# HKUST-Aerial-Robotics/VINS-Mono

Measured on AMD Instinct MI355X. Metric: sliding-window BA solves/sec (Estimator::optimization: 8-iteration dogleg solve + marginalization), higher is better.
Workload: dtype f64; 1 GPU; batch of 256 independent EuRoC-shape windows per step and GPU (K=11 frames, ~150 landmarks, 10 IMU factors, ~600 projection factors, 75-dim marginalization prior, max 8 iterations, MARGIN_OLD marginalization); windows resident in HBM; consecutive steps are issued to 16 HIP streams (independent batches in flight); windows_per_gpu=256, batches_in_flight=16, parallelism=independent batches x1 (no collectives)

## Files before the change

### vins-mono_amd/csrc/ba_host.hip

```cpp
#include "vg_range.h"
#include <hip/hip_runtime.h>
#include <algorithm>
#include <chrono>
#include <cmath>
#include <cstdio>
#include <cstdlib>
#include <cstring>
#include <string>
#include <thread>
#include <vector>
#include "ba_layout.h"
#include "vg_handle.h"
#include "../../include/vinsgpu.h"

struct BaFork { hipStream_t aux; hipEvent_t fork, join; };
extern "C" hipError_t ba_launch_solve(const BaLayout& L, const BaLayout* dL, const BaPtrs& P, int rounds, hipStream_t stream,
                                      hipEvent_t* ev, int* kinds, int* n_launches, const BaFork* fk);
typedef int (*BaAllReduce)(void* user, double* buf, size_t count, void* stream);
extern "C" hipError_t ba_launch_solve_big(const BaLayout& L, const BaLayout* dL, const BaPtrs& P, int rounds, int slack, hipStream_t stream,
                                          BaAllReduce allreduce, void* user, int* hook_rc, hipEvent_t* ev, int* kinds, int* n_launches);
extern "C" hipError_t ba_launch_eval_factors(const BaLayout& L, const BaLayout* dL, const BaPtrs& P, double* proj_r, double* proj_J,
                                            double* imu_r, double* imu_J, double* prior_r, hipStream_t stream);
extern "C" const char* ba_failed_launch();
extern "C" hipError_t ba_prepare_launch();
// ... 184 lines not shown
    }
    L.nbl = L.nbf + L.nig + L.nprw;
    {
        const int nb = L.Kp + L.e + L.t;
        L.ntask = nb * (nb + 1) / 2;
        const int per = BA_ACC_NT / 64;
        const int ng = L.e + L.t, nglob = ng * (ng + 1) / 2;
        L.nba = L.Kp + (ng ? 1 : 0) + (L.ntask - L.Kp - nglob + (L.Lcap + 63) / 64 + per - 1) / per;
    }
    int bigm_doubles = 0;
    {
        int ldc = L.RcPad;
        if ((2 * ldc) % 64 != 32) ldc += 16;
        L.ldc = ldc;
        int o = 0, ob = 0;
        int& oo = L.big ? ob : o;
        L.l_S = o; o += up((L.Rc + 1) * (L.Rc + 2) / 2, 2);
        L.l_XC = 0; L.l_ring = 0; L.l_pinv = 0;
        if (L.big) { L.l_XC = oo; oo += up(9 * L.K, 8) * ldc; }
        else {
            L.l_ring = o; o += 36 * ldc;
        }
        L.l_D = oo; oo += up(81 * L.K, 2);
        L.l_E = oo; oo += up(81 * L.K, 2);
        L.l_dinv = oo; oo += up(9 * L.K, 2);
        L.l_vec = oo; oo += 9 * L.Rpad;
        L.l_red = o; o += 32;
        if (L.big) { L.l_wd = oo; oo += up(std::max(9 * L.K, 162), 2); }
        else L.l_wd = L.l_ring;
        L.l_z = oo; oo += up(36 * L.K, 2);
        if (L.big) { L.l_pmap = oo; oo += up(L.Ncap, 4) / 2; }
        else { L.l_pmap = 0; L.l_pinv = o; o += up(L.R, 4) / 2; }
        if (L.big) { L.l_di = o; o += up(L.Rc + 1, 2); L.l_cz = o; o += 6 * 96; }
        L.l_Sg = 0;
        if (L.big) { L.l_Sg = oo; oo += up((L.Rc + 1) * (L.Rc + 2) / 2, 2); }
        L.lds_solve = o * 8;
        bigm_doubles = ob;
        if (!L.big && L.Rc + 10 - 64 > 32) { h->err = "solve kernel: more column tasks than three wavefronts"; return VG_ERR_UNSUPPORTED; }
        if (!L.big && 36 * ldc < std::max(std::max(L.RcPad * 33, 2 * SV_NT), std::max(9 * L.K, 162))) { h->err = "solve kernel: scratch does not fit the coupling-row ring"; return VG_ERR_UNSUPPORTED; }
        if (L.lds_solve > 160 * 1024) { h->err = "solve kernel LDS carve exceeds 160 KB"; return VG_ERR_UNSUPPORTED; }
        const int nib = std::min(std::min(L.K - 1, BA_IMU_BATCH), L.igs);
        L.lds_lin = 8 * std::max(up(nib * 225, 2) + nib * 480, 5 * L.Ncap);
        L.lds_pro = 8 * BA_NW * (L.imu_info ? 512 : 256);
        if (8 * L.Ncap * L.Ncap <= 128 * 1024) L.lds_pro = std::max(L.lds_pro, 8 * L.Ncap * L.Ncap);
        if (L.lds_lin > 128 * 1024) { h->err = "prior too large for the linearisation kernel"; return VG_ERR_UNSUPPORTED; }
        {
            static const bool env_off = getenv("VG_BA_FUSED") && !strcmp(getenv("VG_BA_FUSED"), "0");
            const bool off = env_off && !h->ba.no_env;
            static const int env_min = getenv("VG_BA_FUSED_MIN") ? atoi(getenv("VG_BA_FUSED_MIN")) : 32;
            const int la_min_windows = h->ba.fused_min >= 0 ? (h->ba.fused_min ? h->ba.fused_min : 1 << 30) : (env_min ? env_min : 1 << 30);
            const int npair = L.Kp * (L.Kp - 1) / 2;
            const int avail = (160 * 1024 - 8192 - 512) / 8;
            const int nstl = up(7 * L.Kp + 9 * L.K + 8, 2);
            int chf = (int)((avail - nstl - npair * 90 - 34 - (64 + 82 + 8 * 80) / 2) / 34.0);
            chf = std::min(chf & ~1, 512);
            L.la_on = (!off && L.nwin >= la_min_windows && !L.big && !L.e && !L.t && L.Kp <= 13 && chf >= 96 && (L.Fcap + chf - 17) / (chf - 16) <= 62) ? 1 : 0;
            L.la_chf = chf; L.la_chq = chf - 16;
            L.la_P = up(chf * 33, 2);
            L.la_key = L.la_P + up(npair * 90, 2);
            L.la_x = up(L.la_key + (2 * chf + 64 + 82 + 8 * 80 + 1) / 2 + 2, 2);
            L.lds_linacc = (L.la_x + nstl) * 8;
        }
        {
            static const int env_max = getenv("VG_BA_SOLVE_W8_BELOW") ? atoi(getenv("VG_BA_SOLVE_W8_BELOW")) : -1;
            const int below = (env_max >= 0 && !h->ba.no_env) ? env_max : 32;
            L.sv_w8 = (!L.big && L.nwin < below) ? 1 : 0;
            L.l_wd8 = L.lds_solve / 8;
            L.lds_solve_w8 = L.lds_solve + 8 * L.RcPad * 33;
            if (L.lds_solve_w8 > 160 * 1024) L.sv_w8 = 0;
        }
    }
    if (L.big) {
        const int nt = (L.Rc + 1 + 15) / 16;
        L.nts = nt * (nt + 1) / 2;
        const int ntri = L.Rc * (L.Rc + 1) / 2;
        L.rb1_T = up(ntri + L.Rc, 2);
        L.rb1_scal = L.rb1_T + up((L.Rc + 1) * (L.Rc + 2) / 2, 2);
        L.rb1_len = L.rb1_scal + RB1_NSCAL;
    }
    int o = 0;
    L.io_hdr = o; o += BA_HDR_INTS;
    L.io_lm_start = o; o += L.Lcap;
    L.io_lm_fbeg = o; o += L.Lcap + 8;
    L.io_fac_i = o; o += L.Fcap;
    L.io_fac_j = o; o += L.Fcap;
    L.io_fac_lm = o; o += L.Fcap;
    L.io_fac_oi = o; o += L.Fcap;
    L.io_fac_oj = o; o += L.Fcap;
    L.io_fac_slot = o; o += L.Fcap;
    L.io_pair_ptr = o; o += up(L.Kp * L.Kp + 1, 8);
    L.io_task_list = o; o += up(L.ntask, 8);
    L.io_imu_valid = o; o += up(L.K, 8);
    L.io_pb_kind = o; o += L.NBcap;
    L.io_pb_idx = o; o += L.NBcap;
    L.io_pb_col = o; o += L.NBcap;
    L.io_pb_off = o; o += L.NBcap;
    L.io_pb_x0off = o; o += L.NBcap;
    L.istride = up(o, 8);
    o = 0;
    L.do_pose = o; o += up(7 * L.Kp, 2);
    L.do_sb = o; o += up(9 * L.K, 2);
    L.do_ex = o; o += 8;
    L.do_td = o; o += 2;
    L.do_lam = o; o += L.Lcap;
    L.do_obs = o; o += L.Ocap * BA_OBS_STRIDE;
    L.do_imu = o; o += (L.K - 1) * BA_IMU_STRIDE;
    L.do_par = o; o += P_NPAR;
    L.dstride = up(o, 8);
    L.pld = std::max(up(6 * L.K + 9 * 2 + 6 + 1, 8), L.Ncap);
    L.po_x0 = 0;
    L.po_r0 = 9 * std::max(up(L.K + 4, 8), L.NBcap);
    L.po_J0 = L.po_r0 + L.pld;
    L.pstride = up(L.po_J0 + L.pld * L.pld, 8);
    o = 0;
    L.so_ctl = o; o += C_NCTL;
    L.so_part = o; o += up(L.nbl, 8);
    L.so_x = o; o += 2 * L.nst;
    L.so_lam = o; o += 2 * L.Lcap;
    L.so_imuU = o; o += up((L.K - 1) * 225, 2);
    L.so_Hp = o; o += L.Ncap * L.Ncap;
    L.so_J0t = o; o += L.Ncap * L.Ncap;
    L.so_rec = o; o += L.Fcap * L.REC;
    L.so_sc = o; o += L.Rpad;
    L.so_sl = o; o += L.Lcap;
    L.so_dg = o; o += L.Rpad + L.Lcap;
    L.so_gt = o; o += L.Rpad + L.Lcap;
    L.so_gn = o; o += L.Rpad + L.Lcap;
    L.so_yl = o; o += L.Lcap;
    L.so_lsc = o; o += L.Lcap;
    L.so_xp = 0;
    if (!L.big) { L.so_xp = o; o += up(9 * L.K, 4) * L.ldc; }
    if (L.big) {
        L.so_bigm = o; o += up(bigm_doubles, 8);
        L.so_dgl = o; o += 2 * L.Lcap;
        L.so_gtl = o; o += 2 * L.Lcap;
    }
    {
        int b = 0;
        L.bo_Sp = b; b += up(L.Rc * (L.Rc + 1) / 2, 2);
        L.bo_gp = b; b += L.RcPad;
        L.bo_h = b; b += L.Lcap;
        L.bo_b = b; b += L.Lcap;
        L.bo_Wt = b; b += L.RcPad * L.Lcap;
        L.bo_imuJ = b; b += (L.K - 1) * 512;
        L.bo_pr = b; b += L.Ncap;
        L.bo_gpr = b; b += L.Ncap;
        L.buf_stride = up(b, 8);
    }
    L.so_buf = o; o += 2 * L.buf_stride;
    L.sstride = up(o, 8);
    L.pl_off = (int)((sizeof(BaLayout) + 255) / 256 * 256);
    L.pl_n = L.big ? 0 : L.Rc * (L.Rc + 1) / 2 + L.Rpad + 2 * 81 * L.K;
    o = 0;
    L.oo_pose = o; o += up(7 * L.Kp, 2);
    L.oo_sb = o; o += up(9 * L.K, 2);
    L.oo_ex = o; o += 8;
    L.oo_td = o; o += 2;
    L.oo_lam = o; o += L.Lcap;
    L.oo_sum = o; o += BA_SUM_DOUBLES;
    L.oo_trace = o; o += 5 * VG_MAX_ITERS + 16;
    L.ostride = up(o, 8);
    L.oi_stride = up(4 + VG_MAX_ITERS, 8);
    L.mcap = up(6 * L.K + 9 * 2 + 6 + 1, 8);
    if (L.mcap > 256) { h->err = "kept dimension of the marginalization beyond the kernel's tables"; return VG_ERR_UNSUPPORTED; }
    const int mcap = L.mcap;
    L.mo_J0 = 0;
    L.mo_r0 = mcap * mcap;
    L.mo_x0 = L.mo_r0 + mcap;
    L.mo_stride = up(L.mo_x0 + (L.K + 4) * 9, 8);
    L.mi_stride = up(8 + 2 * (L.K + 4) + 16, 8);
    L.mg_posmax = up(mcap + 15 + L.Lcap, 2);
    {
        const int nstm = up(16 * L.K + 8 + 1, 2);
        L.mg_cs = up(std::max(std::max(2 * mcap, 3 * (L.mg_posmax / 2 + 2)), 2 * (3 * ((mcap + 2) / 2) + 2) + 2), 2);
        L.mg_cs = std::max(L.mg_cs, std::max(up(5 * mcap + 8, 2), up(L.Lcap + 512, 2)));
        const int fixed = 32 + nstm + BA_MARG_LDS_INTS / 2 + L.mg_cs;
        int ld = mcap + 1;
        while (2 * ld * ld + fixed > 160 * 1024 / 8) ld -= 2;
        L.mg_ld = ld;
        L.mg_lds_bytes = (2 * ld * ld + fixed) * 8;
        if (ld < 8) { h->err = "marginalization LDS carve failed"; return VG_ERR_UNSUPPORTED; }
        const long pm = L.mg_posmax;
        long sdoubles = pm * pm + pm + (long)L.Fcap * 42 + 2 * pm * (mcap + 1) + 2 * pm * pm + 2L * mcap * mcap + 2 * L.Ncap + 480 + L.Lcap + 64 + L.Lcap / 2 + 8;
        L.ms_stride = (int)up((int)sdoubles, 8);
    }
    return VG_OK;
}

struct FacTmp { int i, j, l, oi, oj; };

static int pack_window(vg_handle* h, const BaLayout& L, const vg_ba_problem* p, const PriorRef& pr, int margin, int* ia, double* di, double* hp) {
    const int K = L.K, Kp = L.Kp;
    int* hdr = ia + L.io_hdr;
    for (int o = 0; o < p->n_obs; ++o) {
        double* d = di + L.do_obs + (size_t)o * BA_OBS_STRIDE;
        for (int k = 0; k < 7; ++k) d[k] = p->obs[(size_t)o * 7 + k];
        d[7] = 0.0;
    }
    for (int k = 0; k < p->relo_n; ++k) {
        double* d = di + L.do_obs + (size_t)(p->n_obs + k) * BA_OBS_STRIDE;
        memset(d, 0, sizeof(double) * BA_OBS_STRIDE);
        d[0] = p->relo_xy[2 * k];
// ... 1385 lines not shown
```

### vins-mono_amd/csrc/ba_layout.h

```cpp
#pragma once

#ifndef BA_NT
#define BA_NT 512
#endif
#define BA_NW (BA_NT / 64)
#ifndef SV_NT
#define SV_NT 256
#endif
#define SV_NW (SV_NT / 64)
#define SV_WG_PER_CU (SV_NT <= 256 ? 2 : 1)
#define BA_LIN_NT 256
#define BA_ACC_NT 256
#define BA_MAX_K 13
#define BA_MAX_K_LARGE 40
#define BA_MARG_LDS_INTS 400
#ifndef BA_IMU_BATCH
#define BA_IMU_BATCH 16
#endif
#ifndef BA_IMU_GROUP
#define BA_IMU_GROUP 2
#endif
#define BA_IMU_STRIDE 472
#define BA_OBS_STRIDE 8
#define BA_SUM_DOUBLES 16
#define BA_HDR_INTS 16

enum { H_L = 0, H_F, H_NPRIOR, H_NBLK, H_MAXIT, H_NCHUNK, H_MARGIN, H_STATUS, H_MARGMODE };

enum {
    C_IT = 0, C_NACC, C_NINV, C_TERM, C_STATUS, C_RADIUS, C_MU, C_MUSOLVED, C_REUSE, C_COST, C_XNORM, C_ALPHA, C_GTN2,
    C_GNN2, C_GTGN, C_DNORM, C_MODEL, C_CUR, C_PENDING, C_DONE, C_STEPNORM, C_XNORMC, C_INITCOST, C_SCALED, C_QCAM,
    C_PHASE, C_GNN2C, C_GTGNC, C_STEP2C, C_XN2C,
    C_T0,
    C_TIMEDOUT,
    C_NCTL = 32
};

enum { RB1_COST = 0, RB1_GTL2, RB1_LAM2, RB1_STEP2, RB1_NBIG, RB1_NSCAL = 8 };
enum { RB2_GNN2 = 0, RB2_GTGN, RB2_QL, RB2_NONFIN };
#define BA_BIG_LM_BLOCKS 32
#define BA_BIG_ZERO_BLOCKS 8
#define RB2_LEN (4 * BA_BIG_LM_BLOCKS)

enum { V_G = 0, V_SC, V_DG, V_GT, V_GN, V_U, V_Y, V_T, V_DI, V_NVEC };
struct alignas(16) AsmPlanEntry { int dst, base, imu, cols; };

struct BaLayout {
    int nwin, K, Kp, e, t;
    int Rc, RcPad, R, Rpad;
    int Lcap, Fcap, Ocap, Ncap, NBcap;
    int REC;
    int nbf, nbl, nba, ntask;
    int nig, igs, nprw;
    int nst;
    int imu_info;
    int io_hdr, io_lm_start, io_lm_fbeg, io_fac_i, io_fac_j, io_fac_lm, io_fac_oi, io_fac_oj, io_fac_slot,
        io_pair_ptr, io_task_list, io_imu_valid, io_pb_kind, io_pb_idx, io_pb_col, io_pb_off, io_pb_x0off, istride;
    int do_pose, do_sb, do_ex, do_td, do_lam, do_obs, do_imu, do_par, dstride;
    int po_x0, po_r0, po_J0, pld, pstride;
    int so_ctl, so_part, so_x, so_lam;
    int so_imuU, so_Hp, so_rec;
    int so_J0t;
    int so_sc, so_sl, so_dg, so_gt, so_gn;
    int so_yl, so_lsc;
    int so_xp;
    int so_buf, buf_stride;
    int bo_Sp, bo_gp, bo_h, bo_b, bo_Wt, bo_imuJ, bo_pr, bo_gpr;
    int sstride;
    int oo_pose, oo_sb, oo_ex, oo_td, oo_lam, oo_sum, oo_trace, ostride;
    int oi_stride;
    int mo_J0, mo_r0, mo_x0, mo_stride;
    int mi_stride;
    int ms_stride;
    int mcap, mg_ld, mg_posmax, mg_cs, mg_lds_bytes;
    int l_S, l_XC, l_D, l_E, l_dinv, l_vec, l_red, l_wd, l_z, l_pmap, ldc, lds_solve;
    int l_ring, l_pinv;
    int pl_off, pl_n;
    int lds_lin, lds_pro;
    int la_on, la_chq, la_chf, la_P, la_key, la_x, lds_linacc;
    int sv_w8;
    int l_wd8, lds_solve_w8;
    int pro_split;
    int big;
    int so_bigm;
    int l_di, l_cz;
    int l_Sg;
    int so_dgl, so_gtl;
    int rb1_len, rb1_T, rb1_scal;
    int nts;
};

struct BaPtrs {
    int* iarr;
    double* din;
    double* scr;
    double* out;
    int* iout;
    double* mout;
    int* miout;
    double* mscr;
    double* rb1;
    double* rb2;
    double* pri;
};

enum { P_FOCAL = 0, P_TR, P_ROW, P_GNORM, P_MAXTIME, P_NPAR = 8 };
```

### vins-mono_amd/csrc/ba_pipeline.hip

```cpp
#include <hip/hip_runtime.h>
#include <vector>
#include <mutex>
#include <cstring>
#include <cstdlib>
#include "ba_layout.h"
#include "ba_factors.h"
#include "../../include/vinsgpu.h"

extern __shared__ __attribute__((aligned(16))) char bp_smem[];

#ifdef BA_SOLVE_W8_TU
#undef BA_PROFILE_DETAIL
#undef BA_DEBUG_DUMP
namespace vg_w8 {
#endif

#define NOINL __device__ __noinline__
#define AS_LDS(p) ((lds_d*)(p))
#define AS_LDS_C(p) ((const lds_d*)(p))
#define AS_GLB(p) ((glb_d*)(p))
#define AS_GLB_C(p) ((const glb_d*)(p))
#define AS_GLB_CI(p) ((const glb_i*)(p))
template <bool BIG> struct MovT { typedef lds_d D; typedef lds_i I; };
template <> struct MovT<true> { typedef glb_d D; typedef glb_i I; };
// ... 274 lines not shown
            for (int r = 0; r < 15; ++r) Uo[r * 15 + i] = (i >= r) ? A[i * 15 + r] : 0.0;
        __syncthreads();
    }
}

NOINL void imu_sqrt_info(const Ctx& c_in, int fbeg, int fend) {
    const Ctx c = c_in;
    const BaLayout L = *c.Lp;
    lds_d* A = AS_LDS(LDSB + c.wave * 256);
    const int nimu = fend < L.K - 1 ? fend : L.K - 1;
    const glb_i* valid = AS_GLB_CI(c.ia + L.io_imu_valid);
    const int li = c.lane < 15 ? c.lane : 14;
    for (int base = fbeg; base < nimu; base += BA_NW) {
        const int f = uni(base + c.wave);
        if (!(f < nimu && valid[f])) continue;
        const glb_d* cov = AS_GLB_C(c.di + L.do_imu + f * BA_IMU_STRIDE + IM_COV);
        double a[15];
#pragma unroll
        for (int k = 0; k < 15; ++k) a[k] = cov[li * 15 + k];
#pragma unroll
        for (int j = 14; j >= 0; --j) {
            const double d = sqrt(readlane_f64(a[j], j));
            a[j] = c.lane < j ? a[j] / d : (c.lane == j ? d : a[j]);
#pragma unroll
            for (int kk = 0; kk < j; ++kk) {
                const double ukj = readlane_f64(a[j], kk);
                a[kk] = (c.lane <= kk) ? a[kk] - a[j] * ukj : a[kk];
            }
        }
        if (c.lane < 15) {
#pragma unroll
            for (int k = 0; k < 15; ++k) A[c.lane * 15 + k] = a[k];
        }
        __builtin_amdgcn_wave_barrier();
        glb_d* Uo = AS_GLB(c.sc + L.so_imuU + f * 225);
        if (c.lane < 15) {
            const int j = c.lane;
            double x[15];
#pragma unroll
            for (int i = 14; i >= 0; --i) {
                double s = (i == j) ? 1.0 : 0.0;
#pragma unroll
                for (int k = 14; k > i; --k) s -= (k <= j) ? A[i * 15 + k] * x[k] : 0.0;
                x[i] = (i <= j) ? s / A[i * 15 + i] : 0.0;
            }
#pragma unroll
            for (int i = 0; i < 15; ++i) Uo[i * 15 + j] = x[i];
        }
        __builtin_amdgcn_wave_barrier();
    }
    __syncthreads();
}

#ifndef BA_SOLVE_W8_TU
extern "C" __global__ __launch_bounds__(BA_NT) void ba_prologue_kernel(const BaLayout* __restrict__ Lp, BaPtrs P) {
    const BaLayout& L = *Lp;
    Ctx c;
    ctx_init(c, Lp, P, blockIdx.x);
    double* x = c.sc + L.so_x;
    DP_DECL;
    const bool all = gridDim.y == 1;
    const int part = blockIdx.y, nI = (L.K - 1 + BA_NW - 1) / BA_NW;
    if (all || part == 0)
    {
        double* out = P.out + (size_t)blockIdx.x * L.ostride;
        int* iout = P.iout + (size_t)blockIdx.x * L.oi_stride;
        int* miout = P.miout + (size_t)blockIdx.x * L.mi_stride;
        for (int k = c.tid; k < L.ostride; k += BA_NT) out[k] = 0.0;
        for (int k = c.tid; k < L.oi_stride; k += BA_NT) iout[k] = 0;
        for (int k = c.tid; k < L.mi_stride; k += BA_NT) miout[k] = 0;
    }
    if (all || part == 0) {
        for (int k = c.tid; k < 7 * L.Kp; k += BA_NT) x[k] = c.di[L.do_pose + k];
        for (int k = c.tid; k < 9 * L.K; k += BA_NT) x[7 * L.Kp + k] = c.di[L.do_sb + k];
        if (c.tid < 7) x[7 * L.Kp + 9 * L.K + c.tid] = c.di[L.do_ex + c.tid];
        if (c.tid == 7) x[7 * L.Kp + 9 * L.K + 7] = c.di[L.do_td];
        for (int k = c.tid; k < c.nL; k += BA_NT) c.sc[L.so_lam + k] = c.di[L.do_lam + k];
        if (c.tid < C_NCTL) {
            double v = 0.0;
            if (c.tid == C_RADIUS) v = 1e4;
            if (c.tid == C_MU || c.tid == C_MUSOLVED) v = 1e-8;
            if (c.tid == C_T0) v = (double)wall_clock64();
            c.sc[L.so_ctl + c.tid] = v;
        }
    }
    DP_ADD(40);
    if (all || (part >= 1 && part <= nI)) {
        const int fbeg = all ? 0 : (part - 1) * BA_NW, fend = all ? L.K - 1 : part * BA_NW;
        if (L.imu_info) imu_sqrt_info_ref(c, fbeg, fend);
        else imu_sqrt_info(c, fbeg, fend);
    }
    DP_ADD(41);
    if (c.nprior && (all || part > nI)) {
        const bool do_copy = all || part == nI + 1, do_prod = all || part == nI + 2;
        const int n = c.nprior;
        const double* J0 = c.pri + L.po_J0;
        double* Hp = c.sc + L.so_Hp;
        if (do_copy) {
            double* J0t = c.sc + L.so_J0t;
            for (int wk = c.tid; wk < n * n; wk += BA_NT) { const int r = wk / n, cc = wk % n; J0t[cc * L.Ncap + r] = J0[r * L.pld + cc]; }
        }
        __syncthreads();
        DP_ADD(42);
        if (!do_prod) {
        } else if ((size_t)n * n * 8 <= (size_t)L.lds_pro) {
            double* J0s = LDSB;
            for (int wk = c.tid; wk < n * n; wk += BA_NT) J0s[wk] = J0[(wk / n) * L.pld + wk % n];
            __syncthreads();
            DP_ADD(43);
            const int T = (n + 15) >> 4, ntile = T * (T + 1) / 2, nks = (n + 3) >> 2;
            const int wave = c.tid >> 6, lane = c.tid & 63, li = lane & 15, lk = lane >> 4;
            for (int t = wave; t < ntile; t += BA_NT / 64) {
                int ta, tb;
                tri_decode(t, ta, tb);
                const int ca = 16 * ta + li, cb = 16 * tb + li;
                double4_t acc = (double4_t){0, 0, 0, 0};
                for (int ks = 0; ks < nks; ++ks) {
                    const int r = 4 * ks + lk;
                    const double av = (r < n && ca < n) ? J0s[r * n + ca] : 0.0;
                    const double bv = (r < n && cb < n) ? J0s[r * n + cb] : 0.0;
                    acc = __builtin_amdgcn_mfma_f64_16x16x4f64(av, bv, acc, 0, 0, 0);
                }
#pragma unroll
                for (int q = 0; q < 4; ++q) {
                    const int a = 16 * ta + lk + 4 * q, bb = 16 * tb + li;
                    if (a < n && bb <= a) {
                        Hp[a * L.Ncap + bb] = acc[q];
                    }
                }
            }
        } else {
            const int ld = L.pld;
            for (int wk = c.tid; wk < n * (n + 1) / 2; wk += BA_NT) {
                int a, bb;
                tri_decode(wk, a, bb);
                double s0 = 0.0, s1 = 0.0;
                int r = 0;
                for (; r + 1 < n; r += 2) { s0 += J0[r * ld + a] * J0[r * ld + bb]; s1 += J0[(r + 1) * ld + a] * J0[(r + 1) * ld + bb]; }
                if (r < n) s0 += J0[r * ld + a] * J0[r * ld + bb];
                Hp[a * L.Ncap + bb] = s0 + s1;
            }
        }
    }
    DP_ADD(44);
}
#endif

template <bool JAC>
NOINL double imu_pass(const Ctx& c_in, const double* x_, double* imuJ_, int fbeg, int fend) {
    const Ctx c = c_in;
    const BaLayout L = *c.Lp;
    const int nimu = fend;
    const glb_i* valid = AS_GLB_CI(c.ia + L.io_imu_valid);
    const glb_d* x = AS_GLB_C(x_);
    glb_d* imuJ = AS_GLB(imuJ_);
    const glb_d* gU = AS_GLB_C(c.sc + L.so_imuU);
    const int nb = fend - fbeg < BA_IMU_BATCH ? fend - fbeg : BA_IMU_BATCH;
    double* Us = LDSB;
    double* panels = Us + ((nb * 225 + 1) & ~1);
    double cost = 0.0;
    const int per = nb > BA_NW ? 2 : 1;
    const int half = c.lane >> 5, hl = c.lane & 31;
    for (int f0 = fbeg; f0 < nimu; f0 += nb) {
        const int nf = nimu - f0 < nb ? nimu - f0 : nb;
        for (int k0 = c.tid; k0 < nf * 225; k0 += 8 * BA_NT) {
            double uv[8];
#pragma unroll
            for (int u = 0; u < 8; ++u) { const int k = k0 + u * BA_NT; uv[u] = k < nf * 225 ? gU[f0 * 225 + k] : 0.0; }
#pragma unroll
            for (int u = 0; u < 8; ++u) { const int k = k0 + u * BA_NT; if (k < nf * 225) Us[k] = uv[u]; }
        }
        __syncthreads();
        const int fl = c.wave * per + half;
        const int f = f0 + fl;
        const bool act = fl < nf && half < per && valid[f];
        if (act) {
            const glb_d* pre = AS_GLB_C(c.di + L.do_imu + f * BA_IMU_STRIDE);
            double pi[7], si[9], pj[7], sj[9];
#pragma unroll
            for (int k = 0; k < 7; ++k) { pi[k] = x[7 * f + k]; pj[k] = x[7 * (f + 1) + k]; }
#pragma unroll
            for (int k = 0; k < 9; ++k) { si[k] = x[7 * L.Kp + 9 * f + k]; sj[k] = x[7 * L.Kp + 9 * (f + 1) + k]; }
            const double* U = Us + fl * 225;
            double* panel = panels + fl * 480;
            ImuCtx ic;
            imu_ctx<JAC>(pre, pi, si, pj, sj, c.gnorm, ic);
            double raw[15];
            if (JAC && hl < 30) imu_raw_col(ic, pre, hl, raw);
            else {
#pragma unroll
                for (int q = 0; q < 15; ++q) raw[q] = ic.r[q];
            }
            if (hl <= 30) {
#pragma unroll
                for (int r = 0; r < 15; ++r) {
                    double s = 0.0;
#pragma unroll
// ... 497 lines not shown
    buf[L.bo_b + l] = b;
    int row = 6 * L.Kp;
    if (L.e | L.t) {
        double wex[6] = {0, 0, 0, 0, 0, 0}, wtd = 0.0;
        const int otd = 28 + 12 * L.e;
        for (int f = fb; f < fe; ++f) {
            const double* rec = recs + (size_t)c.ia[L.io_fac_slot + f] * REC;
            const double l0 = rec[24], l1 = rec[25];
            if (L.e) {
#pragma unroll
                for (int k = 0; k < 6; ++k) wex[k] += rec[28 + 2 * k] * l0 + rec[28 + 2 * k + 1] * l1;
            }
            if (L.t) wtd += rec[otd] * l0 + rec[otd + 1] * l1;
        }
        if (L.e) {
#pragma unroll
            for (int k = 0; k < 6; ++k) Wt[(size_t)(col_ex(L) + k) * ldw] = anchor >= 0 ? wex[k] : 0.0;
            row += 6;
        }
        if (L.t) { Wt[(size_t)col_td(L) * ldw] = anchor >= 0 ? wtd : 0.0; row += 1; }
    }
    if (L.big) { Wt[row * ldw] = b; ++row; }
    for (; row < L.RcPad; ++row) Wt[row * ldw] = 0.0;
}

#ifndef BA_SOLVE_W8_TU
extern "C" __global__ __launch_bounds__(BA_ACC_NT) void ba_accumulate_kernel(const BaLayout* __restrict__ Lp, BaPtrs P) {
    const BaLayout& L = *Lp;
    const int bid = blockIdx.x;
    const int xcd = bid & 7, rest = bid >> 3;
    const int bx = rest % L.nba, w = (rest / L.nba) * 8 + xcd;
    if (w >= L.nwin) return;
    Ctx c;
    ctx_init(c, Lp, P, w);
    const double* ctl = c.sc + L.so_ctl;
    if (ctl[C_DONE] != 0.0) return;
    const int which = ((int)ctl[C_CUR]) ^ (ctl[C_PENDING] != 0.0 ? 1 : 0);
    double* buf = lin_buf(c, which);
    const double* recs = c.sc + L.so_rec;
    __shared__ double part[7 * 36 + 4];
    if (bx < L.Kp) { diag_pose_task(c, bx, recs, buf + L.bo_Sp, buf + L.bo_gp, part); return; }
    const int ng = L.e + L.t;
    if (ng && bx == L.Kp) { global_task(c, recs, buf + L.bo_Sp, buf + L.bo_gp, part); return; }
    const int g = (bx - L.Kp - (ng ? 1 : 0)) * (BA_ACC_NT / 64) + c.wave;
    const int nother = L.ntask - L.Kp - ng * (ng + 1) / 2;
    if (g < nother) owner_task(c, c.ia[L.io_task_list + g], c.lane, recs, buf + L.bo_Sp, buf + L.bo_gp);
    else {
        const int l = (g - nother) * 64 + c.lane;
        if (l < L.Lcap) landmark_task(c, l, recs, buf);
    }
}
#endif

#define LA_NT BA_NT
#define LA_RS 33
#define LA_NPW 6
#define LA_MAXP 13
#define LA_QCAP 80
static_assert(LA_QCAP <= 128, "the pair prefix of ba_linacc_proj_kernel takes two pairs per lane of one wavefront");
#define LA_PAIR 90
DEV int wave_scan_incl(int v) {
    v += __builtin_amdgcn_update_dpp(0, v, 0x111, 0xF, 0xF, true);
    v += __builtin_amdgcn_update_dpp(0, v, 0x112, 0xF, 0xF, true);
    v += __builtin_amdgcn_update_dpp(0, v, 0x114, 0xF, 0xF, true);
    v += __builtin_amdgcn_update_dpp(0, v, 0x118, 0xF, 0xF, true);
    const int r0 = __builtin_amdgcn_readlane(v, 15), r1 = __builtin_amdgcn_readlane(v, 31), r2 = __builtin_amdgcn_readlane(v, 47);
    const int row = (int)(threadIdx.x & 63) >> 4;
    return v + (row > 0 ? r0 : 0) + (row > 1 ? r1 : 0) + (row > 2 ? r2 : 0);
}
DEV int la_pair_q(int i, int j, int Kp) { const int d = j - i; return (d - 1) * Kp - (d - 1) * d / 2 + i; }
__device__ __forceinline__ void linacc_body(const BaLayout* __restrict__ Lp, const BaPtrs& P) {
    const BaLayout L = layout_load(Lp);
    Ctx c;
    ctx_init(c, Lp, P, blockIdx.x);
    const double* ctl = c.sc + L.so_ctl;
    if (ctl[C_DONE] != 0.0) return;
    const int which = uni(((int)ctl[C_CUR]) ^ (ctl[C_PENDING] != 0.0 ? 1 : 0));
    const double* x = c.sc + L.so_x + which * L.nst;
    const double* lam = c.sc + L.so_lam + which * L.Lcap;
    glb_d* buf = AS_GLB(lin_buf(c, which));
    const glb_i* ia = AS_GLB_CI(c.ia);
    lds_d* rec = AS_LDS(LDSB);
    lds_d* Pb = AS_LDS(LDSB + L.la_P);
    lds_i* key = (lds_i*)(LDSB + L.la_key);
    lds_i* lstart = key + L.la_chf;
    lds_i* posx = lstart + 64;
    lds_i* pstart = posx + L.la_chf;
    lds_i* wcnt = pstart + LA_QCAP + 2;
    __shared__ double red[2 * (LA_NT / 64)];
    const int Kp = L.Kp, npair = Kp * (Kp - 1) / 2, chq = L.la_chq;
    const int nL = c.nL;
    DP_DECL;
    {
        double share = 0.0;
        if (c.nprior > 0) {
            if (c.nprior * c.nprior <= 12 * LA_NT && 4 * L.Ncap <= 4 * LA_NT && (c.nprior * (c.nprior + 1) + 2 + 5 * L.Ncap) <= L.la_P)
                share = prior_staged(c, L, x, lin_buf(c, which) + L.bo_pr, lin_buf(c, which) + L.bo_gpr, LDSB);
            else
                share = prior_pass(c, x, lin_buf(c, which) + L.bo_pr, lin_buf(c, which) + L.bo_gpr, LDSB);
        }
        DP_ADD(23);
        share += imu_pass<true>(c, x, lin_buf(c, which) + L.bo_imuJ, 0, L.K - 1);
        const double tot_imu = block_sum(red, LA_NT / 64, c.lane, c.wave, share);
        for (int g = c.tid; g < L.nbl - L.nbf; g += LA_NT) c.sc[L.so_part + L.nbf + g] = g == 0 ? tot_imu : 0.0;
        __syncthreads();
        DP_ADD(22);
    }
    lds_d* xs = AS_LDS(LDSB + L.la_x);
    for (int k = c.tid; k < 7 * L.Kp + 9 * L.K + 8; k += LA_NT) xs[k] = AS_GLB_C(x)[k];
    const int nchunk = nL > 0 ? uni(ia[L.io_lm_fbeg + nL - 1] / chq + 1) : 0;
    for (int t = c.tid; t < nL; t += LA_NT) {
        const int cl = ia[L.io_lm_fbeg + t] / chq;
        if (t == 0 || ia[L.io_lm_fbeg + t - 1] / chq != cl) lstart[cl] = t;
    }
    if (c.tid == 0) lstart[nchunk] = nL;
    for (int e = c.tid; e < npair * LA_PAIR; e += LA_NT) Pb[e] = 0.0;
    const bool pair_wave = c.wave < LA_NPW;
    __syncthreads();
    DP_ADD(24);
    int pidx[4];
#pragma unroll
    for (int reg = 0; reg < 4; ++reg) {
        const int row = (c.lane >> 4) + 4 * reg, col = c.lane & 15;
        int idx = -1;
        if (row < 6) {
            if (col <= row) idx = row * (row + 1) / 2 + col;
            else if (col == 13) idx = 78 + row;
        } else if (row < 12) {
            if (col < 6) idx = 42 + (row - 6) * 6 + col;
            else if (col <= row && col < 12) idx = 21 + (row - 6) * (row - 5) / 2 + (col - 6);
            else if (col == 13) idx = 84 + (row - 6);
        }
        pidx[reg] = idx;
    }
    double cost = 0.0;
    for (int ch = 0; ch < nchunk; ++ch) {
        const int l0 = lstart[ch], l1 = lstart[ch + 1];
        const int f0 = ia[L.io_lm_fbeg + l0], f1 = ia[L.io_lm_fbeg + l1];
        const int nf = uni(f1 - f0);
        if (nf > L.la_chf) __builtin_trap();
        ProjIn pin;
        int q = -1, rank = 0;
        if (c.tid < nf) {
            proj_fetch_staged(c, f0 + c.tid, xs, lam, pin);
            q = la_pair_q(pin.i, pin.j, Kp);
        }
        for (int e = c.tid; e < (LA_NT / 64) * LA_QCAP; e += LA_NT) wcnt[e] = 0;
        __syncthreads();
        DP_ADD(45);
        {
            const unsigned long long act = __ballot(q >= 0);
            unsigned long long same = act;
#pragma unroll
            for (int b = 0; b < 7; ++b) {
                const bool bit = q >= 0 && ((q >> b) & 1);
                const unsigned long long mb = __ballot(bit);
                same &= bit ? mb : ~mb;
            }
            const unsigned long long lt = (1ull << c.lane) - 1ull;
            rank = __popcll(same & lt);
            if (q >= 0 && rank == 0) wcnt[c.wave * LA_QCAP + q] = __popcll(same);
        }
        __syncthreads();
        if (c.wave == 0) {
            int cw0[LA_NT / 64], cw1[LA_NT / 64];
            const int p0 = c.lane, p1 = c.lane + 64;
#pragma unroll
            for (int w = 0; w < LA_NT / 64; ++w) {
                cw0[w] = p0 < npair ? wcnt[w * LA_QCAP + p0] : 0;
                cw1[w] = p1 < npair ? wcnt[w * LA_QCAP + p1] : 0;
            }
            int t0 = 0, t1 = 0;
#pragma unroll
            for (int w = 0; w < LA_NT / 64; ++w) { const int a = cw0[w], b = cw1[w]; cw0[w] = t0; cw1[w] = t1; t0 += a; t1 += b; }
            const int i0 = wave_scan_incl(t0);
            const int tot0 = __builtin_amdgcn_readlane(i0, 63);
            const int i1 = wave_scan_incl(t1) + tot0;
            if (p0 < npair) {
                pstart[p0 + 1] = i0;
#pragma unroll
                for (int w = 0; w < LA_NT / 64; ++w) wcnt[w * LA_QCAP + p0] = i0 - t0 + cw0[w];
            }
            if (p1 < npair) {
                pstart[p1 + 1] = i1;
#pragma unroll
                for (int w = 0; w < LA_NT / 64; ++w) wcnt[w * LA_QCAP + p1] = i1 - t1 + cw1[w];
            }
            if (c.lane == 0) pstart[0] = 0;
        }
        __syncthreads();
        DP_ADD(46);
        if (c.tid < nf) {
            const int pos = wcnt[c.wave * LA_QCAP + q] + rank;
            double r[2], Ji[12], Jj[12], Jl[2];
            proj_eval<false, true, false>(pin.pi, pin.pj, pin.ex, pin.lam, pin.oi, pin.oj, 0.0, c.focal, c.tr, c.row, r, Ji, Jj, nullptr, Jl, nullptr);
            const double s = r[0] * r[0] + r[1] * r[1];
            const double sq = sqrt(1.0 / (1.0 + s));
            lds_d* qr = rec + pos * LA_RS;
#pragma unroll
            for (int k = 0; k < 6; ++k) {
                qr[k] = sq * Ji[k]; qr[16 + k] = sq * Ji[6 + k];
                qr[6 + k] = sq * Jj[k]; qr[22 + k] = sq * Jj[6 + k];
            }
            qr[12] = sq * Jl[0]; qr[28] = sq * Jl[1];
            qr[13] = sq * r[0]; qr[29] = sq * r[1];
            key[c.tid] = pin.i * 16 + pin.j;
            posx[c.tid] = pos;
            cost += log1p(s);
        }
        __syncthreads();
        DP_ADD(25);
        if (pair_wave) {
            double4_t acc[LA_MAXP];
#pragma unroll
            for (int k = 0; k < LA_MAXP; ++k) acc[k] = (double4_t){0, 0, 0, 0};
            const int k4 = c.lane >> 4, col = c.lane & 15;
            const int xo = (k4 & 1) * 16 + col;
            const int hi = k4 >> 1;
            const bool incol = col < 14;
#pragma unroll
            for (int k = 0; k < LA_MAXP; ++k) {
                const int qk = c.wave + LA_NPW * k;
                if (qk >= npair) continue;
                const int pb0 = uni(pstart[qk]), pe0 = uni(pstart[qk + 1]);
                DP_ADD(29);
                for (int e = pb0; e < pe0; e += 4) {
                    const int f0r = e + hi, f1r = e + 2 + hi;
                    const double v0 = (f0r < pe0 && incol) ? rec[f0r * LA_RS + xo] : 0.0;
                    const double v1 = (f1r < pe0 && incol) ? rec[f1r * LA_RS + xo] : 0.0;
                    acc[k] = __builtin_amdgcn_mfma_f64_16x16x4f64(v0, v0, acc[k], 0, 0, 0);
                    if (e + 2 < pe0) acc[k] = __builtin_amdgcn_mfma_f64_16x16x4f64(v1, v1, acc[k], 0, 0, 0);
                }
                DP_ADD(30);
            }
#pragma unroll
            for (int k = 0; k < LA_MAXP; ++k) {
                if (c.wave + LA_NPW * k >= npair) continue;
                lds_d* pb = Pb + (c.wave + LA_NPW * k) * LA_PAIR;
                double old4[4];
#pragma unroll
                for (int reg = 0; reg < 4; ++reg) old4[reg] = (ch > 0 && pidx[reg] >= 0) ? pb[pidx[reg]] : 0.0;
#pragma unroll
                for (int reg = 0; reg < 4; ++reg)
                    if (pidx[reg] >= 0) pb[pidx[reg]] = old4[reg] + acc[k][reg];
            }
            DP_ADD(26);
        } else {
            for (int t = c.tid - LA_NPW * 64; t < l1 - l0; t += LA_NT - LA_NPW * 64) {
                const int l = l0 + t;
                glb_d* Wt = buf + L.bo_Wt + l;
                const size_t ldw = L.Lcap;
                const int fb = ia[L.io_lm_fbeg + l] - f0, fe = ia[L.io_lm_fbeg + l + 1] - f0;
                double h = 0.0, b = 0.0, wi[6] = {0, 0, 0, 0, 0, 0};
                const int anchor = fb < fe ? key[fb] >> 4 : -1;
                int jn = 0;
                for (int f = fb; f < fe; ++f) {
                    const lds_d* q = rec + posx[f] * LA_RS;
                    const int j = key[f] & 15;
                    const double l0v = q[12], l1v = q[28];
                    double v[6];
#pragma unroll
                    for (int k = 0; k < 6; ++k) v[k] = q[6 + k] * l0v + q[22 + k] * l1v;
                    h += l0v * l0v + l1v * l1v;
                    b += l0v * q[13] + l1v * q[29];
#pragma unroll
                    for (int k = 0; k < 6; ++k) wi[k] += q[k] * l0v + q[16 + k] * l1v;
                    for (; jn < j; ++jn) {
                        if (jn == anchor) continue;
#pragma unroll
                        for (int k = 0; k < 6; ++k) Wt[(size_t)(6 * jn + k) * ldw] = 0.0;
                    }
#pragma unroll
                    for (int k = 0; k < 6; ++k) Wt[(size_t)(6 * j + k) * ldw] = v[k];
                    jn = j + 1;
                }
                for (; jn < Kp; ++jn) {
                    if (jn == anchor) continue;
#pragma unroll
                    for (int k = 0; k < 6; ++k) Wt[(size_t)(6 * jn + k) * ldw] = 0.0;
                }
                if (anchor >= 0) {
#pragma unroll
                    for (int k = 0; k < 6; ++k) Wt[(size_t)(6 * anchor + k) * ldw] = wi[k];
                }
                for (int row = 6 * Kp; row < L.RcPad; ++row) Wt[(size_t)row * ldw] = 0.0;
                buf[L.bo_h + l] = h;
                buf[L.bo_b + l] = b;
            }
            DP_ADD(27);
        }
        __syncthreads();
    }
    for (int w = c.tid; w < (L.Lcap - nL) * L.RcPad; w += LA_NT) {
        const int row = w / (L.Lcap - nL), l = nL + w % (L.Lcap - nL);
        buf[L.bo_Wt + (size_t)row * L.Lcap + l] = 0.0;
    }
    {
        const int nent = L.Rc * (L.Rc + 1) / 2;
        for (int e = c.tid; e < nent + L.Rc; e += LA_NT) {
            double s = 0.0;
            if (e < nent) {
                int row, colm;
                tri_decode(e, row, colm);
                const int br = row / 6, pr = row - 6 * br, bc = colm / 6, pc = colm - 6 * bc;
                if (br != bc) s = Pb[la_pair_q(bc, br, Kp) * LA_PAIR + 42 + pr * 6 + pc];
                else {
                    const int t = pr * (pr + 1) / 2 + pc;
                    for (int j = br + 1; j < Kp; ++j) s += Pb[la_pair_q(br, j, Kp) * LA_PAIR + t];
                    for (int i = 0; i < br; ++i) s += Pb[la_pair_q(i, br, Kp) * LA_PAIR + 21 + t];
                }
                buf[L.bo_Sp + e] = s;
            } else {
                const int g = e - nent, a = g / 6, k = g - 6 * a;
                for (int j = a + 1; j < Kp; ++j) s += Pb[la_pair_q(a, j, Kp) * LA_PAIR + 78 + k];
                for (int i = 0; i < a; ++i) s += Pb[la_pair_q(i, a, Kp) * LA_PAIR + 84 + k];
                buf[L.bo_gp + g] = s;
            }
        }
    }
    const double tot = block_sum(red, LA_NT / 64, c.lane, c.wave, cost);
    DP_ADD(28);
    if (c.tid < L.nbf) c.sc[L.so_part + c.tid] = c.tid == 0 ? tot : 0.0;
}
#ifndef BA_SOLVE_W8_TU
extern "C" __global__ __launch_bounds__(LA_NT) void ba_linacc_proj_kernel(const BaLayout* __restrict__ Lp, BaPtrs P) { linacc_body(Lp, P); }
#endif

struct SolveLds {
    double *S, *XC, *D, *E, *dinv, *vec, *red, *wd, *z, *di;
    int* pmap;
    int ldc;
    double* ring;
    int* pinv;
    double* xp;
};
DEV void lds_carve(const BaLayout& L, double* sc, SolveLds& m) {
    m.S = LDSB + L.l_S; m.XC = nullptr; m.D = LDSB + L.l_D; m.E = LDSB + L.l_E; m.dinv = LDSB + L.l_dinv;
    m.vec = LDSB + L.l_vec; m.red = LDSB + L.l_red; m.wd = LDSB + L.l_wd; m.z = LDSB + L.l_z;
    m.pmap = nullptr;
    m.ldc = L.ldc;
    m.di = m.vec + V_DI * L.Rpad;
    m.ring = LDSB + L.l_ring; m.pinv = (int*)(LDSB + L.l_pinv); m.xp = sc + L.so_xp;
}
DEV void big_carve(const BaLayout& L, double* sc, SolveLds& m) {
    double* hb = sc + L.so_bigm;
    m.S = LDSB + L.l_S; m.red = LDSB + L.l_red; m.di = LDSB + L.l_di;
    m.XC = hb + L.l_XC; m.D = hb + L.l_D; m.E = hb + L.l_E; m.dinv = hb + L.l_dinv;
    m.vec = hb + L.l_vec; m.wd = hb + L.l_wd; m.z = hb + L.l_z;
// ... 2886 lines not shown
```

Before: 185,600 solves/s.

## Precompute per-window projection chunk plan in prologue and drop per-iteration Wt zeroing

```diff
diff --git a/vins-mono_amd/csrc/ba_host.hip b/vins-mono_amd/csrc/ba_host.hip
--- a/vins-mono_amd/csrc/ba_host.hip
+++ b/vins-mono_amd/csrc/ba_host.hip
@@ -260,14 +260,15 @@
             const int npair = L.Kp * (L.Kp - 1) / 2;
             const int avail = (160 * 1024 - 8192 - 512) / 8;
             const int nstl = up(7 * L.Kp + 9 * L.K + 8, 2);
-            int chf = (int)((avail - nstl - npair * 90 - 34 - (64 + 82 + 8 * 80) / 2) / 34.0);
-            chf = std::min(chf & ~1, 512);
-            L.la_on = (!off && L.nwin >= la_min_windows && !L.big && !L.e && !L.t && L.Kp <= 13 && chf >= 96 && (L.Fcap + chf - 17) / (chf - 16) <= 62) ? 1 : 0;
+            int chf = (int)((avail - nstl - L.Lcap - npair * 90 - 34 - (2 * 64 + 82) / 2) / 34.0);
+            chf = std::min(std::max(chf, 0) & ~1, 512);
+            L.la_on = (!off && L.nwin >= la_min_windows && !L.big && !L.e && !L.t && L.Kp <= 13 && chf >= 96 && (L.Fcap + chf - 17) / (chf - 16) <= LA_MAXCH) ? 1 : 0;
             L.la_chf = chf; L.la_chq = chf - 16;
             L.la_P = up(chf * 33, 2);
             L.la_key = L.la_P + up(npair * 90, 2);
-            L.la_x = up(L.la_key + (2 * chf + 64 + 82 + 8 * 80 + 1) / 2 + 2, 2);
-            L.lds_linacc = (L.la_x + nstl) * 8;
+            L.la_x = up(L.la_key + (2 * chf + 2 * 64 + LA_PL_PSLD + 1) / 2 + 2, 2);
+            L.lds_linacc = (L.la_x + nstl + L.Lcap) * 8;
+            if (L.la_on && L.lds_linacc > 160 * 1024 - 8192 - 512) { h->err = "fused projection kernel: LDS carve exceeds its budget"; return VG_ERR_UNSUPPORTED; }
         }
         {
             static const int env_max = getenv("VG_BA_SOLVE_W8_BELOW") ? atoi(getenv("VG_BA_SOLVE_W8_BELOW")) : -1;
@@ -356,6 +357,15 @@
         L.buf_stride = up(b, 8);
     }
     L.so_buf = o; o += 2 * L.buf_stride;
+    L.so_plan = 0; L.pl_ps = 0; L.pl_meta = 0; L.pl_obs = 0;
+    if (!L.big) {
+        o = up(o, 2);
+        L.so_plan = o;
+        L.pl_ps = LA_PL_HDR;
+        L.pl_meta = L.pl_ps + LA_MAXCH * LA_PL_PSLD;
+        L.pl_obs = up(L.pl_meta + 2 * L.Fcap, 4) / 2;
+        o += L.pl_obs + 4 * L.Fcap;
+    }
     L.sstride = up(o, 8);
     L.pl_off = (int)((sizeof(BaLayout) + 255) / 256 * 256);
     L.pl_n = L.big ? 0 : L.Rc * (L.Rc + 1) / 2 + L.Rpad + 2 * 81 * L.K;
diff --git a/vins-mono_amd/csrc/ba_layout.h b/vins-mono_amd/csrc/ba_layout.h
--- a/vins-mono_amd/csrc/ba_layout.h
+++ b/vins-mono_amd/csrc/ba_layout.h
@@ -24,6 +24,12 @@
 #define BA_OBS_STRIDE 8
 #define BA_SUM_DOUBLES 16
 #define BA_HDR_INTS 16
+#define LA_PL_NCH 0
+#define LA_PL_LST 4
+#define LA_PL_FST 68
+#define LA_PL_HDR 132
+#define LA_PL_PSLD 82
+#define LA_MAXCH 62
 
 enum { H_L = 0, H_F, H_NPRIOR, H_NBLK, H_MAXIT, H_NCHUNK, H_MARGIN, H_STATUS, H_MARGMODE };
 
@@ -78,6 +84,7 @@
     int pl_off, pl_n;
     int lds_lin, lds_pro;
     int la_on, la_chq, la_chf, la_P, la_key, la_x, lds_linacc;
+    int so_plan, pl_ps, pl_meta, pl_obs;
     int sv_w8;
     int l_wd8, lds_solve_w8;
     int pro_split;
diff --git a/vins-mono_amd/csrc/ba_pipeline.hip b/vins-mono_amd/csrc/ba_pipeline.hip
--- a/vins-mono_amd/csrc/ba_pipeline.hip
+++ b/vins-mono_amd/csrc/ba_pipeline.hip
@@ -350,6 +350,116 @@
     __syncthreads();
 }
 
+#define LA_NT BA_NT
+#define LA_RS 33
+#define LA_NPW 6
+#define LA_MAXP 13
+#define LA_QCAP 80
+static_assert(LA_QCAP <= 128, "the pair prefix of la_plan_build takes two pairs per lane of one wavefront");
+static_assert(LA_QCAP + 2 <= LA_PL_PSLD, "a row of the plan's pair-start table holds pstart[0 .. LA_QCAP]");
+#define LA_PAIR 90
+DEV int wave_scan_incl(int v) {
+    v += __builtin_amdgcn_update_dpp(0, v, 0x111, 0xF, 0xF, true);
+    v += __builtin_amdgcn_update_dpp(0, v, 0x112, 0xF, 0xF, true);
+    v += __builtin_amdgcn_update_dpp(0, v, 0x114, 0xF, 0xF, true);
+    v += __builtin_amdgcn_update_dpp(0, v, 0x118, 0xF, 0xF, true);
+    const int r0 = __builtin_amdgcn_readlane(v, 15), r1 = __builtin_amdgcn_readlane(v, 31), r2 = __builtin_amdgcn_readlane(v, 47);
+    const int row = (int)(threadIdx.x & 63) >> 4;
+    return v + (row > 0 ? r0 : 0) + (row > 1 ? r1 : 0) + (row > 2 ? r2 : 0);
+}
+DEV int la_pair_q(int i, int j, int Kp) { const int d = j - i; return (d - 1) * Kp - (d - 1) * d / 2 + i; }
+
+DEV void la_plan_build(const Ctx& c, const BaLayout& L) {
+    const glb_i* ia = AS_GLB_CI(c.ia);
+    const glb_d* obs = AS_GLB_C(c.di + L.do_obs);
+    glb_i* pl = (glb_i*)(c.sc + L.so_plan);
+    glb_d* pobs = AS_GLB(c.sc + L.so_plan + L.pl_obs);
+    lds_i* wcnt = (lds_i*)LDSB;
+    lds_i* lst = wcnt + (LA_NT / 64) * LA_QCAP;
+    const int Kp = L.Kp, npair = Kp * (Kp - 1) / 2, chq = L.la_chq, nL = c.nL;
+    const int nchunk = nL > 0 ? uni(ia[L.io_lm_fbeg + nL - 1] / chq + 1) : 0;
+    for (int t = c.tid; t < nL; t += LA_NT) {
+        const int cl = ia[L.io_lm_fbeg + t] / chq;
+        if (t == 0 || ia[L.io_lm_fbeg + t - 1] / chq != cl) lst[cl] = t;
+    }
+    if (c.tid == 0) { lst[nchunk] = nL; pl[LA_PL_NCH] = nchunk; }
+    __syncthreads();
+    if (c.tid <= nchunk) {
+        const int l = lst[c.tid];
+        pl[LA_PL_LST + c.tid] = l;
+        pl[LA_PL_FST + c.tid] = ia[L.io_lm_fbeg + l];
+    }
+    for (int ch = 0; ch < nchunk; ++ch) {
+        const int l0 = lst[ch], l1 = lst[ch + 1];
+        const int f0 = uni(ia[L.io_lm_fbeg + l0]), f1 = uni(ia[L.io_lm_fbeg + l1]);
+        const int nf = uni(f1 - f0);
+        const int f = f0 + c.tid;
+        const bool own = c.tid < nf && c.tid < L.la_chf;
+        int fi = 0, fj = 0, fl = 0, q = -1, rank = 0;
+        double ov[4] = {0, 0, 0, 0};
+        if (own) {
+            fi = ia[L.io_fac_i + f]; fj = ia[L.io_fac_j + f]; fl = ia[L.io_fac_lm + f];
+            const int oi = ia[L.io_fac_oi + f], oj = ia[L.io_fac_oj + f];
+            ov[0] = obs[oi * BA_OBS_STRIDE]; ov[1] = obs[oi * BA_OBS_STRIDE + 1];
+            ov[2] = obs[oj * BA_OBS_STRIDE]; ov[3] = obs[oj * BA_OBS_STRIDE + 1];
+            q = la_pair_q(fi, fj, Kp);
+        }
+        for (int e = c.tid; e < (LA_NT / 64) * LA_QCAP; e += LA_NT) wcnt[e] = 0;
+        __syncthreads();
+        {
+            const unsigned long long act = __ballot(q >= 0);
+            unsigned long long same = act;
+#pragma unroll
+            for (int b = 0; b < 7; ++b) {
+                const bool bit = q >= 0 && ((q >> b) & 1);
+                const unsigned long long mb = __ballot(bit);
+                same &= bit ? mb : ~mb;
+            }
+            const unsigned long long lt = (1ull << c.lane) - 1ull;
+            rank = __popcll(same & lt);
+            if (q >= 0 && rank == 0) wcnt[c.wave * LA_QCAP + q] = __popcll(same);
+        }
+        __syncthreads();
+        if (c.wave == 0) {
+            glb_i* pstart = pl + L.pl_ps + ch * LA_PL_PSLD;
+            int cw0[LA_NT / 64], cw1[LA_NT / 64];
+            const int p0 = c.lane, p1 = c.lane + 64;
+#pragma unroll
+            for (int w = 0; w < LA_NT / 64; ++w) {
+                cw0[w] = p0 < npair ? wcnt[w * LA_QCAP + p0] : 0;
+                cw1[w] = p1 < npair ? wcnt[w * LA_QCAP + p1] : 0;
+            }
+            int t0 = 0, t1 = 0;
+#pragma unroll
+            for (int w = 0; w < LA_NT / 64; ++w) { const int a = cw0[w], b = cw1[w]; cw0[w] = t0; cw1[w] = t1; t0 += a; t1 += b; }
+            const int i0 = wave_scan_incl(t0);
+            const int tot0 = __builtin_amdgcn_readlane(i0, 63);
+            const int i1 = wave_scan_incl(t1) + tot0;
+            if (p0 < npair) {
+                pstart[p0 + 1] = i0;
+#pragma unroll
+                for (int w = 0; w < LA_NT / 64; ++w) wcnt[w * LA_QCAP + p0] = i0 - t0 + cw0[w];
+            }
+            if (p1 < npair) {
+                pstart[p1 + 1] = i1;
+#pragma unroll
+                for (int w = 0; w < LA_NT / 64; ++w) wcnt[w * LA_QCAP + p1] = i1 - t1 + cw1[w];
+            }
+            if (c.lane == 0) pstart[0] = 0;
+        }
+        __syncthreads();
+        if (own) {
+            const int pos = wcnt[c.wave * LA_QCAP + q] + rank;
+            pl[L.pl_meta + 2 * f] = (fi * 16 + fj) | (pos << 8);
+            pl[L.pl_meta + 2 * f + 1] = fl;
+#pragma unroll
+            for (int k = 0; k < 4; ++k) pobs[4 * (size_t)f + k] = ov[k];
+        }
+        __syncthreads();
+    }
+    __syncthreads();
+}
+
 #ifndef BA_SOLVE_W8_TU
 extern "C" __global__ __launch_bounds__(BA_NT) void ba_prologue_kernel(const BaLayout* __restrict__ Lp, BaPtrs P) {
     const BaLayout& L = *Lp;
@@ -383,6 +493,8 @@
         }
     }
     DP_ADD(40);
+    if (L.la_on && (all || part == 0)) la_plan_build(c, L);
+    DP_ADD(47);
     if (all || (part >= 1 && part <= nI)) {
         const int fbeg = all ? 0 : (part - 1) * BA_NW, fend = all ? L.K - 1 : part * BA_NW;
         if (L.imu_info) imu_sqrt_info_ref(c, fbeg, fend);
@@ -441,6 +553,14 @@
         }
     }
     DP_ADD(44);
+    if (L.la_on && (all || part == 0)) {
+        const int nw = L.RcPad * L.Lcap;
+        for (int b = 0; b < 2; ++b) {
+            glb_d* Wt = AS_GLB(c.sc + L.so_buf + (size_t)b * L.buf_stride + L.bo_Wt);
+            for (int k = c.tid; k < nw; k += BA_NT) Wt[k] = 0.0;
+        }
+        DP_ADD(48);
+    }
 }
 #endif
 
@@ -1044,23 +1164,6 @@
 }
 #endif
 
-#define LA_NT BA_NT
-#define LA_RS 33
-#define LA_NPW 6
-#define LA_MAXP 13
-#define LA_QCAP 80
-static_assert(LA_QCAP <= 128, "the pair prefix of ba_linacc_proj_kernel takes two pairs per lane of one wavefront");
-#define LA_PAIR 90
-DEV int wave_scan_incl(int v) {
-    v += __builtin_amdgcn_update_dpp(0, v, 0x111, 0xF, 0xF, true);
-    v += __builtin_amdgcn_update_dpp(0, v, 0x112, 0xF, 0xF, true);
-    v += __builtin_amdgcn_update_dpp(0, v, 0x114, 0xF, 0xF, true);
-    v += __builtin_amdgcn_update_dpp(0, v, 0x118, 0xF, 0xF, true);
-    const int r0 = __builtin_amdgcn_readlane(v, 15), r1 = __builtin_amdgcn_readlane(v, 31), r2 = __builtin_amdgcn_readlane(v, 47);
-    const int row = (int)(threadIdx.x & 63) >> 4;
-    return v + (row > 0 ? r0 : 0) + (row > 1 ? r1 : 0) + (row > 2 ? r2 : 0);
-}
-DEV int la_pair_q(int i, int j, int Kp) { const int d = j - i; return (d - 1) * Kp - (d - 1) * d / 2 + i; }
 __device__ __forceinline__ void linacc_body(const BaLayout* __restrict__ Lp, const BaPtrs& P) {
     const BaLayout L = layout_load(Lp);
     Ctx c;
@@ -1076,11 +1179,13 @@
     lds_d* Pb = AS_LDS(LDSB + L.la_P);
     lds_i* key = (lds_i*)(LDSB + L.la_key);
     lds_i* lstart = key + L.la_chf;
-    lds_i* posx = lstart + 64;
+    lds_i* fstart = lstart + 64;
+    lds_i* posx = fstart + 64;
     lds_i* pstart = posx + L.la_chf;
-    lds_i* wcnt = pstart + LA_QCAP + 2;
+    const glb_i* pl = (const glb_i*)(c.sc + L.so_plan);
+    const glb_d* pobs = AS_GLB_C(c.sc + L.so_plan + L.pl_obs);
     __shared__ double red[2 * (LA_NT / 64)];
-    const int Kp = L.Kp, npair = Kp * (Kp - 1) / 2, chq = L.la_chq;
+    const int Kp = L.Kp, npair = Kp * (Kp - 1) / 2;
     const int nL = c.nL;
     DP_DECL;
     {
@@ -1099,13 +1204,11 @@
         DP_ADD(22);
     }
     lds_d* xs = AS_LDS(LDSB + L.la_x);
+    lds_d* lams = xs + ((7 * L.Kp + 9 * L.K + 8 + 1) & ~1);
     for (int k = c.tid; k < 7 * L.Kp + 9 * L.K + 8; k += LA_NT) xs[k] = AS_GLB_C(x)[k];
-    const int nchunk = nL > 0 ? uni(ia[L.io_lm_fbeg + nL - 1] / chq + 1) : 0;
-    for (int t = c.tid; t < nL; t += LA_NT) {
-        const int cl = ia[L.io_lm_fbeg + t] / chq;
-        if (t == 0 || ia[L.io_lm_fbeg + t - 1] / chq != cl) lstart[cl] = t;
-    }
-    if (c.tid == 0) lstart[nchunk] = nL;
+    for (int k = c.tid; k < nL; k += LA_NT) lams[k] = AS_GLB_C(lam)[k];
+    if (c.tid < 128) lstart[c.tid] = pl[LA_PL_LST + c.tid];
+    const int nchunk = uni(pl[LA_PL_NCH]);
     for (int e = c.tid; e < npair * LA_PAIR; e += LA_NT) Pb[e] = 0.0;
     const bool pair_wave = c.wave < LA_NPW;
     __syncthreads();
@@ -1128,64 +1231,24 @@
     double cost = 0.0;
     for (int ch = 0; ch < nchunk; ++ch) {
         const int l0 = lstart[ch], l1 = lstart[ch + 1];
-        const int f0 = ia[L.io_lm_fbeg + l0], f1 = ia[L.io_lm_fbeg + l1];
+        const int f0 = fstart[ch], f1 = fstart[ch + 1];
         const int nf = uni(f1 - f0);
         if (nf > L.la_chf) __builtin_trap();
-        ProjIn pin;
-        int q = -1, rank = 0;
+        if (c.tid <= npair) pstart[c.tid] = pl[L.pl_ps + ch * LA_PL_PSLD + c.tid];
         if (c.tid < nf) {
-            proj_fetch_staged(c, f0 + c.tid, xs, lam, pin);
-            q = la_pair_q(pin.i, pin.j, Kp);
-        }
-        for (int e = c.tid; e < (LA_NT / 64) * LA_QCAP; e += LA_NT) wcnt[e] = 0;
-        __syncthreads();
-        DP_ADD(45);
-        {
-            const unsigned long long act = __ballot(q >= 0);
-            unsigned long long same = act;
-#pragma unroll
-            for (int b = 0; b < 7; ++b) {
-                const bool bit = q >= 0 && ((q >> b) & 1);
-                const unsigned long long mb = __ballot(bit);
-                same &= bit ? mb : ~mb;
-            }
-            const unsigned long long lt = (1ull << c.lane) - 1ull;
-            rank = __popcll(same & lt);
-            if (q >= 0 && rank == 0) wcnt[c.wave * LA_QCAP + q] = __popcll(same);
-        }
-        __syncthreads();
-        if (c.wave == 0) {
-            int cw0[LA_NT / 64], cw1[LA_NT / 64];
-            const int p0 = c.lane, p1 = c.lane + 64;
-#pragma unroll
-            for (int w = 0; w < LA_NT / 64; ++w) {
-                cw0[w] = p0 < npair ? wcnt[w * LA_QCAP + p0] : 0;
-                cw1[w] = p1 < npair ? wcnt[w * LA_QCAP + p1] : 0;
-            }
-            int t0 = 0, t1 = 0;
-#pragma unroll
-            for (int w = 0; w < LA_NT / 64; ++w) { const int a = cw0[w], b = cw1[w]; cw0[w] = t0; cw1[w] = t1; t0 += a; t1 += b; }
-            const int i0 = wave_scan_incl(t0);
-            const int tot0 = __builtin_amdgcn_readlane(i0, 63);
-            const int i1 = wave_scan_incl(t1) + tot0;
-            if (p0 < npair) {
-                pstart[p0 + 1] = i0;
-#pragma unroll
-                for (int w = 0; w < LA_NT / 64; ++w) wcnt[w * LA_QCAP + p0] = i0 - t0 + cw0[w];
-            }
-            if (p1 < npair) {
-                pstart[p1 + 1] = i1;
-#pragma unroll
-                for (int w = 0; w < LA_NT / 64; ++w) wcnt[w * LA_QCAP + p1] = i1 - t1 + cw1[w];
-            }
-            if (c.lane == 0) pstart[0] = 0;
-        }
-        __syncthreads();
-        DP_ADD(46);
-        if (c.tid < nf) {
-            const int pos = wcnt[c.wave * LA_QCAP + q] + rank;
+            const int f = f0 + c.tid;
+            const int m0 = pl[L.pl_meta + 2 * f], fl = pl[L.pl_meta + 2 * f + 1];
+            const double oi[2] = {pobs[4 * (size_t)f], pobs[4 * (size_t)f + 1]}, oj[2] = {pobs[4 * (size_t)f + 2], pobs[4 * (size_t)f + 3]};
+            const int kij = m0 & 255, pos = m0 >> 8;
+            const int fi = kij >> 4, fj = kij & 15;
+            double pi[7], pj[7], ex[8];
+#pragma unroll
+            for (int k = 0; k < 7; ++k) { pi[k] = xs[7 * fi + k]; pj[k] = xs[7 * fj + k]; }
+#pragma unroll
+            for (int k = 0; k < 8; ++k) ex[k] = xs[7 * L.Kp + 9 * L.K + k];
+            const double lamv = lams[fl];
             double r[2], Ji[12], Jj[12], Jl[2];
-            proj_eval<false, true, false>(pin.pi, pin.pj, pin.ex, pin.lam, pin.oi, pin.oj, 0.0, c.focal, c.tr, c.row, r, Ji, Jj, nullptr, Jl, nullptr);
+            proj_eval<false, true, false>(pi, pj, ex, lamv, oi, oj, 0.0, c.focal, c.tr, c.row, r, Ji, Jj, nullptr, Jl, nullptr);
             const double s = r[0] * r[0] + r[1] * r[1];
             const double sq = sqrt(1.0 / (1.0 + s));
             lds_d* qr = rec + pos * LA_RS;
@@ -1196,7 +1259,7 @@
             }
             qr[12] = sq * Jl[0]; qr[28] = sq * Jl[1];
             qr[13] = sq * r[0]; qr[29] = sq * r[1];
-            key[c.tid] = pin.i * 16 + pin.j;
+            key[c.tid] = kij;
             posx[c.tid] = pos;
             cost += log1p(s);
         }
@@ -1245,7 +1308,6 @@
                 const int fb = ia[L.io_lm_fbeg + l] - f0, fe = ia[L.io_lm_fbeg + l + 1] - f0;
                 double h = 0.0, b = 0.0, wi[6] = {0, 0, 0, 0, 0, 0};
                 const int anchor = fb < fe ? key[fb] >> 4 : -1;
-                int jn = 0;
                 for (int f = fb; f < fe; ++f) {
                     const lds_d* q = rec + posx[f] * LA_RS;
                     const int j = key[f] & 15;
@@ -1257,35 +1319,19 @@
                     b += l0v * q[13] + l1v * q[29];
 #pragma unroll
                     for (int k = 0; k < 6; ++k) wi[k] += q[k] * l0v + q[16 + k] * l1v;
-                    for (; jn < j; ++jn) {
-                        if (jn == anchor) continue;
-#pragma unroll
-                        for (int k = 0; k < 6; ++k) Wt[(size_t)(6 * jn + k) * ldw] = 0.0;
-                    }
 #pragma unroll
                     for (int k = 0; k < 6; ++k) Wt[(size_t)(6 * j + k) * ldw] = v[k];
-                    jn = j + 1;
-                }
-                for (; jn < Kp; ++jn) {
-                    if (jn == anchor) continue;
-#pragma unroll
-                    for (int k = 0; k < 6; ++k) Wt[(size_t)(6 * jn + k) * ldw] = 0.0;
                 }
                 if (anchor >= 0) {
 #pragma unroll
                     for (int k = 0; k < 6; ++k) Wt[(size_t)(6 * anchor + k) * ldw] = wi[k];
                 }
-                for (int row = 6 * Kp; row < L.RcPad; ++row) Wt[(size_t)row * ldw] = 0.0;
                 buf[L.bo_h + l] = h;
                 buf[L.bo_b + l] = b;
             }
             DP_ADD(27);
         }
         __syncthreads();
-    }
-    for (int w = c.tid; w < (L.Lcap - nL) * L.RcPad; w += LA_NT) {
-        const int row = w / (L.Lcap - nL), l = nL + w % (L.Lcap - nL);
-        buf[L.bo_Wt + (size_t)row * L.Lcap + l] = 0.0;
     }
     {
         const int nent = L.Rc * (L.Rc + 1) / 2;
```

Result: faster. 189,100 solves/s (median of 6 runs) (+1.9%).
